# TIXhjq/ML_Function

Measured on AMD Instinct MI355X. Metric: samples/sec fwd+bwd xDeepFM-CIN B=4096,F=39,K=16, higher is better.
Workload: dtype f32

## Files before the change

### ml_function_amd/csrc/cin.hip

```cpp
#include "cin_kernels.h"
#include "cin_tail.h"
#include "cin_launch.h"
#include "cin_qtail.h"
#include "cin_qsplit.h"
#include "cin_qmerge.h"

#include <stdlib.h>

namespace fil {

struct CinShape {
  int B, F, K, L;
  int H[kCinMaxL];
  int Hp(int l) const { return l == 0 ? F : H[l - 1]; }
  int HS(int l) const { return 128 * cdiv(H[l], 128); }
  int xps(int l) const { return l == 0 ? F : HS(l - 1); }
  long M() const { return (long)B * K; }
  int JT() const { return cin_jt_of(F); }
  int HSmax() const {
    int h = 0;
    for (int l = 0; l < L; ++l) h = std::max(h, HS(l));
    return h;
  }
};
// ... 224 lines not shown
  return w;
}
static int dz_periods(const CinShape& s, int l) { return cdiv(s.Hp(l), cin_dz_h_per_period(s.JT())); }
static size_t wz_floats(const CinShape& s) {
  const int jts = cin_jt_sym(s.F);
  size_t w = ((size_t)cdiv(s.F, cin_dz_h_per_period(jts)) * cin_dz_tiles_per_period(jts) + 1) * 32 * s.HS(0);
  w = std::max(w, (size_t)s.F * (s.F / 2 + 1) * s.H[0]);
  for (int l = 0; l < s.L; ++l) w = std::max(w, ((size_t)dz_periods(s, l) * cin_dz_tiles_per_period(s.JT()) + 1) * 32 * s.HS(l));
  return w;
}
static int pool_chunks(const CinShape& s, int l) { return std::max(chunks_of(s.H[l]), l > 0 ? chunks_of(s.H[l - 1]) : 1); }
static size_t fwd_ws_bytes(const CinShape& s) {
  size_t t = 0;
  for (int l = 0; l < s.L; ++l) t += align_up((size_t)pool_chunks(s, l) * s.M() * sizeof(float), 256);
  t += align_up((size_t)s.Hp(s.L - 1) * s.F * sizeof(float), 256);
  t += align_up(wf_floats(s) * sizeof(float), 256);
  t += align_up((size_t)kCinMaxH * sizeof(float), 256);
  t += align_up(cin_x2_floats(s.M(), cin_x2_len(s.F)) * sizeof(float), 256);
  t += align_up((size_t)chunks_of(s.H[0]) * s.F * 2 * cin_jt_sym(s.F) * 128 * sizeof(float), 256);
  t += align_up(qsplit_wb_bytes(s), 256);
  return t;
}
static size_t dw_part_floats(const CinShape& s) {
  size_t pmax = 0;
  for (int l = 0; l < s.L; ++l) pmax = std::max(pmax, (size_t)dw_plan(s.M(), s.Hp(l) * s.F, s.H[l]).splits * s.Hp(l) * s.F * s.H[l]);
  const int csym = s.F * (s.F / 2 + 1);
  pmax = std::max(pmax, (size_t)dw_plan(s.M(), csym, s.H[0]).splits * csym * s.H[0]);
  pmax = std::max(pmax, (size_t)dw_plan(s.M(), csym + s.F, s.H[0]).splits * (csym + s.F) * s.H[0]);
  if (s.L == 3) pmax = std::max(pmax, (size_t)cin_dwq_plan(s.M(), csym + s.F, cu_count()).pairs * (csym + s.F) * 256);
  if (s.L == 3) pmax = std::max(pmax, (size_t)cin_dwqb_plan(s.M(), csym + s.F, cu_count()).splits * (csym + s.F) * 256);
  pmax = std::max(pmax, (size_t)dw_plan(s.M(), s.Hp(s.L - 1), s.F).splits * s.Hp(s.L - 1) * s.F);
  pmax = std::max(pmax, (size_t)dw_plan(s.M(), s.F, s.Hp(s.L - 1)).splits * s.Hp(s.L - 1) * s.F);
  const TailGeom g = tail_geom(s);
  if (g.on) {
    pmax = std::max(pmax, (size_t)tail_dw_plan(s.M(), g.C1).splits * g.C1 * g.JP + (size_t)cdiv(g.Cp, kTailPc) * g.Hq * s.F);
  }
  return pmax;
}
static size_t bwd_ws_bytes(const CinShape& s) {
  const size_t LK = (size_t)s.L * s.K;
  const size_t M = (size_t)s.M();
  size_t t = 0;
  t += align_up((size_t)s.B * LK * sizeof(float), 256);
  t += 2 * align_up(M * s.HSmax() * sizeof(float), 256);
  t += align_up(dw_part_floats(s) * sizeof(float), 256);
  const size_t nblk = (size_t)cdiv(std::max(1, s.B), kHeadChunk);
  const size_t ncol = (M + kColRows - 1) / kColRows;
  t += align_up(std::max(ncol * s.HSmax(), nblk * (LK + 1)) * sizeof(float), 256);
  const size_t cl = (size_t)std::max(s.Hp(s.L - 1), s.L == 3 ? s.H[0] : 0) * s.F;
  t += 2 * align_up(cl * sizeof(float), 256);
  t += align_up(wz_floats(s) * sizeof(float), 256);
  t += 2 * align_up(M * s.F * sizeof(float), 256);
  t += align_up((size_t)s.F * s.F * kCinMaxH * sizeof(float), 256);
  t += align_up(((M + 255) / 256 + 1) * kQtConst * sizeof(float), 256);
  t += align_up(((M + 255) / 256) * (LK + 1) * sizeof(float), 256);
  t += 2 * align_up(qsplit_wzb_bytes(s), 256);
  return t;
}

template <typename KernelT>
static void allow_lds(KernelT kernel, size_t sh) {
  if (sh > 48 * 1024) (void)hipFuncSetAttribute(reinterpret_cast<const void*>(kernel), hipFuncAttributeMaxDynamicSharedMemorySize, (int)sh);
}

}

using namespace fil;

extern "C" size_t fil_cin_saved_bytes(int B, int F, int K, int L, const int* H) {
  CinShape s;
  if (check_shape("fil_cin_saved_bytes", B, F, K, L, H, s) != FIL_OK || B == 0) return 0;
  return saved_bytes(s);
}

extern "C" size_t fil_cin_fwd_workspace_bytes(int B, int F, int K, int L, const int* H) {
  CinShape s;
  if (check_shape("fil_cin_fwd_workspace_bytes", B, F, K, L, H, s) != FIL_OK || B == 0) return 0;
  return fwd_ws_bytes(s);
}

extern "C" size_t fil_cin_bwd_workspace_bytes(int B, int F, int K, int L, const int* H) {
  CinShape s;
  if (check_shape("fil_cin_bwd_workspace_bytes", B, F, K, L, H, s) != FIL_OK || B == 0) return 0;
  return bwd_ws_bytes(s);
}

extern "C" int fil_cin_grad_ready_points(int B, int F, int K, int L, const int* H, int mode, int* point) {
  CinShape s;
  if (int rc = check_shape("fil_cin_grad_ready_points", B, F, K, L, H, s)) return rc;
  if (point == nullptr || mode < 0 || mode > 1023) return fail(FIL_ERR_ARG, "fil_cin_grad_ready_points: point == NULL or mode %d out of range", mode);
  if ((mode & kCinRetiredBits) != 0) return fail(FIL_ERR_UNSUPPORTED, "fil_cin_grad_ready_points: mode %d holds a retired bit (2: the split-bf16 experiment)", mode);
  if (B == 0) {
    for (int i = 0; i <= L; ++i) point[i] = 0;
    return 1;
  }
  int pt = 0, l = L - 1;
  point[L] = pt++;
  if (qmerge_used(s, mode, CinTune(mode))) {
    point[0] = point[L] = 0;
    pt = 1;
    point[1] = point[2] = pt++;
    return pt;
  }
  if (tail_used(s, mode)) {
    point[L - 1] = point[L - 2] = pt++;
    l = L - 3;
  }
// ... 337 lines not shown
    mode |= bits;
  }
  const bool xt_in = (mode & FIL_CIN_X_TRANSPOSED) != 0;
  const CinTune tune(mode);
  const bool tail = tail_used(s, mode);
  const bool qtail = qtail_used(s, mode, tune);
  const bool qmerge = qmerge_used(s, mode, tune);
  const bool qsplit = qsplit_used(s, mode, tune);
  const int qnp = qsplit_planes(mode);
  const TailGeom tg = tail_geom(s);
  mode &= 1;
  FIL_CIN_CHECK_ARG(W && dW && dbias);
  hipStream_t st = (hipStream_t)stream;
  const size_t LK = (size_t)L * K;
  auto ready = [&](int slot) {
    if (grad_ready_events != nullptr && grad_ready_events[slot] != nullptr) (void)hipEventRecord((hipEvent_t)grad_ready_events[slot], st);
  };
  if (B == 0) {
    for (int l = 0; l < L; ++l) {
      (void)hipMemsetAsync(dW[l], 0, (size_t)s.Hp(l) * F * H[l] * sizeof(float), st);
      (void)hipMemsetAsync(dbias[l], 0, (size_t)H[l] * sizeof(float), st);
    }
    if (output_dim == 1) {
      (void)hipMemsetAsync(ddense_w, 0, LK * sizeof(float), st);
      (void)hipMemsetAsync(ddense_b, 0, sizeof(float), st);
    }
    for (int l = 0; l <= L; ++l) ready(l);
    return FIL_OK;
  }
  FIL_CIN_CHECK_ARG(g && dx && saved && (x || !xt_in));
  FIL_CIN_CHECK_ARG(output_dim != 1 || (dense_w && pooled && ddense_w && ddense_b));
  if (workspace == nullptr || workspace_bytes < bwd_ws_bytes(s))
    return fail(FIL_ERR_WORKSPACE, "fil_cin_bwd: workspace %zu < %zu bytes", workspace_bytes, bwd_ws_bytes(s));
  const long M = s.M();
  const int JT = s.JT();
  Carver ws(workspace);
  float* dP = ws.take<float>((size_t)B * LK);
  float* Gbuf[2];
  Gbuf[0] = ws.take<float>((size_t)M * s.HSmax());
  Gbuf[1] = ws.take<float>((size_t)M * s.HSmax());
  float* part = ws.take<float>(dw_part_floats(s));
  const int nblk = cdiv(B, kHeadChunk);
  const int ncol = (int)((M + kColRows - 1) / kColRows);
  float* small = ws.take<float>(std::max((size_t)ncol * s.HSmax(), (size_t)nblk * (LK + 1)));
  const size_t cl = (size_t)s.Hp(L - 1) * F;
  const size_t cl_buf = (size_t)std::max(s.Hp(L - 1), L == 3 ? H[0] : 0) * F;
  float* wsum = ws.take<float>(cl_buf);
  float* vlast = ws.take<float>(cl_buf);
  float* Wz = ws.take<float>(wz_floats(s));
  float* dxT = ws.take<float>((size_t)M * F);
  float* gx0T = ws.take<float>((size_t)M * F);
  float* qt_dT = ws.take<float>((size_t)F * F * kCinMaxH);
  const int qt_ndc = (int)((M + 255) / 256);
  float* qt_dcpart = ws.take<float>((size_t)(qt_ndc + 1) * kQtConst);
  float* qt_hpart = ws.take<float>((size_t)qt_ndc * (LK + 1));
  u32x4* Wzb1 = reinterpret_cast<u32x4*>(ws.take<unsigned char>(qsplit_wzb_bytes(s)));
  u32x4* Wzb2 = reinterpret_cast<u32x4*>(ws.take<unsigned char>(qsplit_wzb_bytes(s)));

  Carver sv(const_cast<float*>(saved));
  const float* xT_own = sv.take<float>((size_t)M * F);
  const float* xT = xt_in ? x : xT_own;
  const float* maps[kCinMaxL];
  const float *tailY = nullptr, *tailUz = nullptr, *tailWsum = nullptr;
  const float *qtR = nullptr, *qtT = nullptr, *qtWsumL = nullptr, *qtCvec = nullptr, *qtWsumP = nullptr, *qtWsnP = nullptr, *qtWzT = nullptr;
  if (qtail) {
    maps[0] = sv.take<float>((size_t)M * s.HS(0));
    const float* q = sv.take<float>(qtail_saved_floats(s));
    qtR = q;
    qtT = qtR + (size_t)M * s.HS(0);
    qtWsumL = qtT + (size_t)F * F * H[0];
    qtCvec = qtWsumL + (size_t)H[1] * F;
    qtWsumP = qtCvec + 128;
    qtWsnP = qtWsumP + (size_t)H[0] * F;
    qtWzT = qtWsnP + qtail_wsn_floats(s);
  } else if (tail) {
    for (int l = 0; l < tg.p; ++l) maps[l] = sv.take<float>((size_t)M * s.HS(l));
    tailY = sv.take<float>((size_t)M * tg.JP);
    tailUz = sv.take<float>(tg.uz_floats + tg.uf_floats);
    tailWsum = sv.take<float>((size_t)tg.Hq * F);
  } else {
    for (int l = 0; l + 1 < L; ++l) maps[l] = sv.take<float>((size_t)M * s.HS(l));
  }

  const float* dPsrc = g;
  if (output_dim == 1 && qmerge) {
    dPsrc = dP;
  } else if (output_dim == 1) {
    ProfScope ps("cin_head_bwd", st);
    hipLaunchKernelGGL(cin_head_bwd_kernel, dim3(nblk), dim3(256), 0, st, g, dense_w, pooled, dP, small, B, (int)LK, kHeadChunk);
    if (!tail) hipLaunchKernelGGL(cin_reduce_kernel, dim3(cdiv((int)LK + 1, 64)), dim3(256), 0, st, small, ddense_w, (long)(LK + 1), nblk, ddense_b, (long)LK);
    FIL_CHECK_LAUNCH();
    dPsrc = dP;
  }
  if (!tail) ready(L);

  int cur = 0;
  int ltop = L - 1;
  bool dx_started = false;
  bool have_gx0 = false;
  bool wz_prepacked = false;
  bool qm_joined = false;
  if (qmerge) {
    const int p = tg.p, lL = L - 1, Hpp = tg.Hpp, Hq = tg.Hq, HS0 = s.HS(0);
    FIL_CIN_CHECK_ARG(bias && W[0] && W[p] && W[lL] && bias[p] && dW[0] && dW[p] && dW[lL] && dbias[0] && dbias[p] && dbias[lL]);
    const float* xpT = maps[p - 1];
    const int xps = s.xps(p);
    const float* dPp = dPsrc + (size_t)p * K;
// ... 15 lines not shown
      allow_lds(cin_qtail_xe_kernel<3>, sh);
      allow_lds(cin_qtail_xe_kernel<1>, sh);
      const int np = (int)std::min<long>(((long)tiles0 * 32 * HS0 + 255) / 256, 1024);
      const int nq2 = qsplit ? 2 * std::min(cdiv(tiles0 * 512, 256), 256) : 0;
      if (qnp == 1)
        hipLaunchKernelGGL(cin_qtail_xe_kernel<1>, dim3(qt_ndc + np + nq2), dim3(kXeThreads), sh, st, xT, dPL, dPp, (int)LK, K, xe, qt_dcpart, (int)M, F,
                           qt_ndc, output_dim == 1 ? g : nullptr, dense_w, pooled, dP, qt_hpart, (int)LK, lL, p, W[0], Wz, H[0], JTs, HS0, tiles0, np, qtT,
                           Hpp, Wzb1, Wzb2);
      else
        hipLaunchKernelGGL(cin_qtail_xe_kernel<3>, dim3(qt_ndc + np + nq2), dim3(kXeThreads), sh, st, xT, dPL, dPp, (int)LK, K, xe, qt_dcpart, (int)M, F,
                           qt_ndc, output_dim == 1 ? g : nullptr, dense_w, pooled, dP, qt_hpart, (int)LK, lL, p, W[0], Wz, H[0], JTs, HS0, tiles0, np, qtT,
                           Hpp, Wzb1, Wzb2);
    }
    FIL_CHECK_LAUNCH();
    {
      ProfScope ps("cin_last_bwd", st, 6.0 * (double)M * Hpp * F);
      cin_launch_last_bwd2(st, JT, xT, xpT, xps, qtWsumP, qtWsnP, dPp, (int)LK, dPprev, Gbuf[cur], HS0, dxT, (int)M, F, K, Hpp, qtR, HS0, dPL, small);
    }
    FIL_CHECK_LAUNCH();
    int dw_parts = 0;
    {
      ProfScope ps("cin_bwd_dw_q", st, algo1 + algo_tail, gemm_flops(M, 1, Cl, H[0]) + gemm_flops(M, 1, Cl, Hpp));
      if (qsplit) {
        const DwqbPlan bp = cin_dwqb_plan(M, Cl + F, cu_count());
        cin_launch_dwq_b(st, qnp, bp, Gbuf[cur], xpT, HS0, xe, XE, part, (int)M, F, symD);
        dw_parts = bp.splits;
      } else {
        const bool f4 = knobs().dwfold4 != 0;
        const DwqPlan dp = f4 ? cin_dwq_plan4(M, Cl + F, cu_count()) : cin_dwq_plan(M, Cl + F, cu_count());
        if (f4)
          hipLaunchKernelGGL((cin_dwq_kernel<kDwqDepth, 4>), dim3((dp.wgs + 7) / 8 * 8), dim3(kDwqThreads), 0, st, Gbuf[cur], xpT, HS0, xe, XE, part, (int)M, F,
                             symD, dp.rows_per_split, dp.splits, dp.ncol_full, dp.rem, dp.wgs_full, dp.wgs);
        else
          hipLaunchKernelGGL((cin_dwq_kernel<kDwqDepth, 2>), dim3((dp.wgs + 7) / 8 * 8), dim3(kDwqThreads), 0, st, Gbuf[cur], xpT, HS0, xe, XE, part, (int)M, F,
                             symD, dp.rows_per_split, dp.splits, dp.ncol_full, dp.rem, dp.wgs_full, dp.wgs);
        dw_parts = dp.pairs;
      }
    }
    FIL_CHECK_LAUNCH();
    {
      ProfScope ps("cin_reduce_dw", st);
      const int nb1 = cdiv(H[0], 64);
      const int nh = output_dim == 1 ? cdiv((int)LK + 1, 64) : 0;
      hipLaunchKernelGGL(cin_reduce_expand_q_kernel, dim3((Cl + F + 3) / 4 + nb1 + nh), dim3(256), 0, st, part, dw_parts, F, symD, H[0], Hpp, dW[0], qt_dT,
                         vlast, small, ncol, dbias[0], nb1, qt_hpart, qt_ndc, (int)LK, ddense_w, ddense_b);
    }
    FIL_CHECK_LAUNCH();
    ready(L);
    ready(0);
    {
      ProfScope ps("cin_tail_params", st);
      const size_t sh = cin_qtail_params_lds(F, Hq);
      allow_lds(cin_qtail_params_kernel, sh);
      float* dcfin = qt_dcpart + (size_t)qt_ndc * kQtConst;
      hipLaunchKernelGGL(cin_qtail_params_kernel, dim3(2 * Hpp + 1), dim3(256), sh, st, W[p], qtWsumL, qt_dT, vlast, dW[p], part, Hpp, F, Hq, qt_dcpart, qt_ndc,
                         dcfin);
      hipLaunchKernelGGL(cin_qtail_fill_kernel, dim3(cdiv(Hq * F, kQtFillCols)), dim3(kQtFillThreads), 0, st, part, Hpp, dcfin, bias[p], qtWsumL, dW[lL], dbias[p], dbias[lL], F, Hq,
                         tg.HL);
    }
    FIL_CHECK_LAUNCH();
    ready(lL);
    ready(p);
    const int NHMAX = HS0 / 2;
    if (NHMAX == 64 && knobs().dz2 != 0) {
      ProfScope ps("cin_bwd_dz_q", st, algo1 + algo_tail, gemm_flops(M, 1, Cl, H[0]) + gemm_flops(M, 1, Cl, Hpp));
      bool split_done = false;
      if (qsplit) {
        split_done = cin_launch_dz2_b(st, qnp, JTs, Gbuf[cur], xpT, HS0, dPL, (int)LK, K, Wzb1, Wzb2, xT, dxT, 1, (int)M, F, H[0], Hpp, periods, dx, qtCvec);
      }
      if (!split_done &&
          !cin_launch_dz2(st, JTs, Gbuf[cur], xpT, HS0, dPL, (int)LK, K, Wz, qtWzT, xT, dxT, 1, (int)M, F, H[0], Hpp, periods, dx, qtCvec))
        return fail(FIL_ERR_UNSUPPORTED, "fil_cin_bwd: no two-pass data-gradient kernel for JT=%d (F=%d)", JTs, F);
      qm_joined = true;
    } else {
      const bool two_waves = NHMAX == 64 && cin_dzs_two_waves(JTs) && tune.mb_forced != 2 && knobs().dzs_mb != 2;
      const int MBs = two_waves ? 1 : tune.mb_rows(M);
      const int ks = MBs != 1 ? 1 : tune.ksplit(M);
      const dim3 zgrid(ks == 4 ? cdiv((int)M, 32) : cdiv((int)M, 128 * MBs));
      {
        ProfScope ps("cin_bwd_dz_tail", st, algo_tail, gemm_flops(M, 1, Cl, Hpp));
        cin_launch_dz3_sym(st, MBs, JTs, NHMAX, zgrid, xpT, HS0, qtWzT, xT, gxR, dxR, 0, (int)M, F, Hpp, periods, ks);
      }
      FIL_CHECK_LAUNCH();
      {
        ProfScope ps("cin_bwd_dz_l1", st, algo1, gemm_flops(M, 1, Cl, H[0]));
        cin_launch_dz3_sym(st, MBs, JTs, NHMAX, zgrid, Gbuf[cur], HS0, Wz, xT, gx0T, dxT, 1, (int)M, F, H[0], periods, ks);
      }
      have_gx0 = true;
    }
    FIL_CHECK_LAUNCH();
    dx_started = true;
    ltop = -1;
  } else if (qtail) {
    const int p = tg.p, lL = L - 1, Hpp = tg.Hpp, Hq = tg.Hq, HS0 = s.HS(0);
    FIL_CIN_CHECK_ARG(bias && W[p] && W[lL] && bias[p] && dW[p] && dW[lL] && dbias[p] && dbias[lL]);
    const float* xpT = maps[p - 1];
    const int xps = s.xps(p);
    const float* dPp = dPsrc + (size_t)p * K;
    const float* dPL = dPsrc + (size_t)lL * K;
    const float* dPprev = dPsrc + (size_t)(p - 1) * K;
    const double algo = gemm_flops(M, Hpp, F, Hq) + gemm_flops(M, Hq, F, tg.HL);
    float* xs = Gbuf[1];
    float* gxR = xs + (size_t)M * (F + 1);
    float* dxR = gxR + (size_t)M * F;
    {
      ProfScope ps("cin_tail_a", st, (double)M * (F + 64) * sizeof(float));
      const size_t sh = (size_t)256 * (F + 3) * sizeof(float);
      allow_lds(cin_qtail_scale_kernel, sh);
      const int nh = output_dim == 1 ? cdiv((int)LK + 1, 64) : 0;
      FIL_CIN_CHECK_ARG(W[0]);
      const int JTs0 = cin_jt_sym(F);
      const int tiles0 = cdiv(F, cin_dz_h_per_period(JTs0)) * cin_dz_tiles_per_period(JTs0) + 1;
      const int np = (int)std::min<long>(((long)tiles0 * 32 * HS0 + 255) / 256, 1024);
      hipLaunchKernelGGL(cin_qtail_scale_kernel, dim3(qt_ndc + nh + np), dim3(256), sh, st, xT, dPL, dPp, (int)LK, K, xs, qt_dcpart, (int)M, F, qt_ndc, small,
                         ddense_w, ddense_b, (int)LK, nblk, nh, W[0], Wz, H[0], JTs0, HS0, tiles0);
      wz_prepacked = true;
    }
    FIL_CHECK_LAUNCH();
    ready(L);
    {
      ProfScope ps("cin_last_bwd", st, 6.0 * (double)M * Hpp * F);
      cin_launch_last_bwd2(st, JT, xT, xpT, xps, qtWsumP, qtWsnP, dPp, (int)LK, dPprev, Gbuf[cur], HS0, dxT, (int)M, F, K, Hpp, qtR, HS0, dPL, small);
    }
    FIL_CHECK_LAUNCH();
    const int symD = F / 2 + 1, Cl = F * symD;
    const int JTs = cin_jt_sym(F);
    {
      ProfScope ps("cin_bwd_dw_tail", st, algo, gemm_flops(M, 1, Cl, Hpp));
      const int parts = launch_dw3(st, dw_plan(M, Cl + F, Hpp), xpT, HS0, xT, xs, F + 1, part, M, F, F, Hpp, symD, F);
      const long nW = (long)Cl * Hpp, pstride = (long)(Cl + F) * Hpp;
      hipLaunchKernelGGL(cin_reduce_expand_sym_kernel, dim3((int)((nW + 63) / 64) + cdiv(F * Hpp, 64)), dim3(256), 0, st, part, qt_dT, F, symD, Hpp, parts,
                         pstride, vlast, (long)F * Hpp);
    }
    FIL_CHECK_LAUNCH();
    {
      ProfScope ps("cin_tail_params", st);
      const size_t sh = cin_qtail_params_lds(F, Hq);
      allow_lds(cin_qtail_params_kernel, sh);
      float* dcfin = qt_dcpart + (size_t)qt_ndc * kQtConst;
      hipLaunchKernelGGL(cin_qtail_params_kernel, dim3(2 * Hpp + 1), dim3(256), sh, st, W[p], qtWsumL, qt_dT, vlast, dW[p], part, Hpp, F, Hq, qt_dcpart, qt_ndc,
                         dcfin);
      hipLaunchKernelGGL(cin_qtail_fill_kernel, dim3(cdiv(Hq * F, kQtFillCols)), dim3(kQtFillThreads), 0, st, part, Hpp, dcfin, bias[p], qtWsumL, dW[lL], dbias[p], dbias[lL], F, Hq,
                         tg.HL);
    }
    FIL_CHECK_LAUNCH();
    ready(lL);
    ready(p);
    {
      const int periods = cdiv(F, cin_dz_h_per_period(JTs));
      ProfScope ps("cin_bwd_dz_tail", st, algo, gemm_flops(M, 1, Cl, Hpp));
      const int NHMAX = HS0 / 2;
      const bool two_waves = NHMAX == 64 && cin_dzs_two_waves(JTs) && tune.mb_forced != 2 && knobs().dzs_mb != 2;
      const int MBs = two_waves ? 1 : tune.mb_rows(M);
      const int ks = MBs != 1 ? 1 : tune.ksplit(M);
      cin_launch_dz3_sym(st, MBs, JTs, NHMAX, dim3(ks == 4 ? cdiv((int)M, 32) : cdiv((int)M, 128 * MBs)), xpT, HS0, qtWzT, xT, gxR, dxR, 0, (int)M, F, Hpp,
                         periods, ks);
    }
    FIL_CHECK_LAUNCH();
    dx_started = true;
    ltop = p - 1;
  } else if (tail) {
    const int p = tg.p, lL = L - 1;
    FIL_CIN_CHECK_ARG(bias && W[p] && W[lL] && bias[p] && dW[p] && dW[lL] && dbias[p] && dbias[lL]);
    const float* xpT = maps[p - 1];
    const int xps = s.xps(p);
    const double algo = gemm_flops(M, tg.Hpp, F, tg.Hq) + gemm_flops(M, tg.Hq, F, tg.HL);
    float* Apk = Gbuf[1];
    wz_prepacked = p == 1 && tune.sym && F >= 2;
    {
      ProfScope ps("cin_tail_a", st, (double)M * (F + 64) * sizeof(float));
      const int na = (int)std::min<long>((M * 16 * tg.NCB + 255) / 256, 4096);
      const int nh = output_dim == 1 ? cdiv((int)LK + 1, 64) : 0;
      int np = 0, JTs = 0, tiles0 = 0;
      if (wz_prepacked) {
        FIL_CIN_CHECK_ARG(W[0]);
        JTs = cin_jt_sym(F);
        tiles0 = cdiv(F, cin_dz_h_per_period(JTs)) * cin_dz_tiles_per_period(JTs) + 1;
        np = (int)std::min<long>(((long)tiles0 * 32 * s.HS(0) + 255) / 256, 1024);
      }
      hipLaunchKernelGGL(cin_tail_pre_kernel, dim3(na + nh + np), dim3(256), 0, st, xT, dPsrc, (int)LK, K, p, lL, Apk, (int)M, F, tg.NCB, na, small,
                         ddense_w, ddense_b, (int)LK, nblk, nh, W[0], Wz, H[0], JTs, s.HS(0), tiles0);
    }
    FIL_CHECK_LAUNCH();
    ready(L);
    const TailDwPlan tp = tail_dw_plan(M, tg.C1);
    {
      ProfScope ps("cin_bwd_dw_tail", st, algo, 2.0 * (double)M * tg.C1 * (F + 2));
      TailDwArgs a{Apk, xT, xpT, xps, part, (int)M, F, tg.Hpp, tg.JP, tp.rows_per_split, tp.blocks_x, tp.blocks_x * tp.splits, knobs().tail_settle != 0};
      cin_launch_tail_dw(st, tg.NCB, a);
    }
    FIL_CHECK_LAUNCH();
    {
      ProfScope ps("cin_tail_params", st);
      const int nblk_p = cdiv(tg.Cp, kTailPc);
      const int ldb = (tg.Hq + 3) & ~3;
      const size_t sh = ((size_t)(F + 1) * ldb + (size_t)tg.JP * (kTailPc + 4) + (size_t)kTailPc * ldb) * sizeof(float);
// ... 159 lines not shown
```

### ml_function_amd/csrc/cin_qtail.h

```cpp
#pragma once
#include "cin_kernels.h"
#include "cin_split.h"

namespace fil {

__device__ __forceinline__ void qt_stage(const float* __restrict__ src, float* dst, int n) {
  for (int i0 = threadIdx.x; i0 < n; i0 += 8 * 256) {
    float v[8];
#pragma unroll
    for (int u = 0; u < 8; ++u) v[u] = i0 + u * 256 < n ? src[i0 + u * 256] : 0.f;
#pragma unroll
    for (int u = 0; u < 8; ++u)
      if (i0 + u * 256 < n) dst[i0 + u * 256] = v[u];
  }
}
__device__ __forceinline__ void qt_stage_rows(const float* __restrict__ src, float* dst, int rows, int cols, int ld) {
  const int n = rows * cols;
  for (int i0 = threadIdx.x; i0 < n; i0 += 8 * 256) {
    float v[8];
#pragma unroll
    for (int u = 0; u < 8; ++u) v[u] = i0 + u * 256 < n ? src[i0 + u * 256] : 0.f;
#pragma unroll
    for (int u = 0; u < 8; ++u) {
      const int i = i0 + u * 256;
// ... 313 lines not shown
    }
  }
}

static __global__ __launch_bounds__(256) void cin_qtail_scale_kernel(const float* __restrict__ xT, const float* __restrict__ dPL,
                                                                     const float* __restrict__ dPp, int ldp, int K, float* __restrict__ xs,
                                                                     float* __restrict__ dcpart, int M, int F, int nscale,
                                                                     const float* __restrict__ hpart, float* __restrict__ ddw, float* __restrict__ ddb,
                                                                     int LK, int nhp, int nhead, const float* __restrict__ W0, float* __restrict__ Wz,
                                                                     int H0, int JTs, int HS0, int tiles0) {
  extern __shared__ __attribute__((aligned(16))) float smem[];
  if ((int)blockIdx.x >= nscale + nhead) {
    cin_pack_wz_sym_body(W0, Wz, F, H0, JTs, HS0, tiles0, blockIdx.x - nscale - nhead, gridDim.x - nscale - nhead);
    return;
  }
  if ((int)blockIdx.x >= nscale) {
    cin_reduce_body(hpart, ddw, (long)LK + 1, nhp, ddb, (long)LK, blockIdx.x - nscale);
    return;
  }
  const int ld = F + 3;
  const long m = (long)blockIdx.x * 256 + threadIdx.x;
  float* row = smem + threadIdx.x * ld;
  if (m < M) {
    const long b = m / K;
    const float dl = dPL[b * ldp + (m - b * K)], dp = dPp[b * ldp + (m - b * K)];
    for (int f = 0; f < F; ++f) {
      const float v = xT[m * F + f] * dl;
      xs[m * (F + 1) + f] = v;
      row[f] = v;
    }
    xs[m * (F + 1) + F] = dp;
    row[F] = dl;
    row[F + 1] = dp;
  } else {
    for (int f = 0; f < F + 2; ++f) row[f] = 0.f;
  }
  __syncthreads();
  __shared__ float cs[4][64];
  {
    const int f = threadIdx.x & 63, q = threadIdx.x >> 6;
    float t0 = 0.f, t1 = 0.f;
    if (f < F + 2) {
      for (int rr = 64 * q; rr < 64 * q + 64; rr += 2) {
        t0 += smem[rr * ld + f];
        t1 += smem[(rr + 1) * ld + f];
      }
    }
    cs[q][f] = t0 + t1;
  }
  __syncthreads();
  if (threadIdx.x < F + 2) dcpart[(long)blockIdx.x * kQtConst + threadIdx.x] = (cs[0][threadIdx.x] + cs[1][threadIdx.x]) + (cs[2][threadIdx.x] + cs[3][threadIdx.x]);
}

static __global__ __launch_bounds__(256) void cin_qtail_params_kernel(const float* __restrict__ Wp, const float* __restrict__ wsumL,
                                                                      const float* __restrict__ dT, const float* __restrict__ vT,
                                                                      float* __restrict__ dWp, float* __restrict__ partL, int Hpp, int F, int Hq,
                                                                      const float* __restrict__ dcpart, int ndc, float* __restrict__ dcfin) {
  extern __shared__ __attribute__((aligned(16))) float smem[];
  if ((int)blockIdx.x == 2 * Hpp) {
    float* red = smem;
    const int lane = threadIdx.x & 63, wave = threadIdx.x >> 6;
    float a0 = 0.f, a1 = 0.f, a2 = 0.f, a3 = 0.f;
    if (lane < F + 2) {
      int p = wave;
      for (; p + 60 < ndc; p += 64) {
        float u[16];
#pragma unroll
        for (int e = 0; e < 16; ++e) u[e] = dcpart[(long)(p + 4 * e) * kQtConst + lane];
#pragma unroll
        for (int e = 0; e < 16; e += 4) {
          a0 += u[e];
          a1 += u[e + 1];
          a2 += u[e + 2];
          a3 += u[e + 3];
        }
      }
      for (; p < ndc; p += 4) a0 += dcpart[(long)p * kQtConst + lane];
    }
    red[wave * 64 + lane] = (a0 + a1) + (a2 + a3);
    __syncthreads();
    if (wave == 0) dcfin[lane] = (red[lane] + red[64 + lane]) + (red[128 + lane] + red[192 + lane]);
    return;
  }
  const int h = blockIdx.x >> 1, phase = blockIdx.x & 1;
  const int FT = (F + 31) & ~31, HT = (Hq + 31) & ~31, FK16 = (F + 15) & ~15, ldd = FT + 1;
  float* dt = smem;
  float* op = dt + FT * ldd;
  const int nop = phase == 0 ? HT * ldd : FK16 * HT;
  const float* osrc = phase == 0 ? wsumL : Wp + (long)h * F * Hq;
  const int ocols = phase == 0 ? F : Hq, old = phase == 0 ? ldd : HT, on = F * Hq;
  const float rF = 1.f / (float)F, rO = 1.f / (float)ocols;
  constexpr int ND = 8, NO = 24;
  float dv[ND], ov[NO];
#pragma unroll
  for (int u = 0; u < ND; ++u) dv[u] = (int)threadIdx.x + u * 256 < F * F ? dT[(long)(threadIdx.x + u * 256) * Hpp + h] : 0.f;
#pragma unroll
  for (int u = 0; u < NO; ++u) ov[u] = (int)threadIdx.x + u * 256 < on ? osrc[threadIdx.x + u * 256] : 0.f;
  for (int i = threadIdx.x; i < FT * ldd + nop; i += 256) smem[i] = 0.f;
  __syncthreads();
  auto put_dt = [&](int i, float v) {
    const int fp = (int)(((float)i + 0.5f) * rF);
    dt[fp * ldd + (i - fp * F)] = v;
  };
  auto put_op = [&](int i, float v) {
    const int rr = (int)(((float)i + 0.5f) * rO);
    op[rr * old + (i - rr * ocols)] = v;
  };
#pragma unroll
  for (int u = 0; u < ND; ++u)
    if ((int)threadIdx.x + u * 256 < F * F) put_dt(threadIdx.x + u * 256, dv[u]);
#pragma unroll
  for (int u = 0; u < NO; ++u)
    if ((int)threadIdx.x + u * 256 < on) put_op(threadIdx.x + u * 256, ov[u]);
  for (int i = threadIdx.x + ND * 256; i < F * F; i += 256) put_dt(i, dT[(long)i * Hpp + h]);
  for (int i = threadIdx.x + NO * 256; i < on; i += 256) put_op(i, osrc[i]);
  __syncthreads();
  const int lane = threadIdx.x & 63, wave = threadIdx.x >> 6, r = lane & 31, half = lane >> 5;
  const bool two = F > 32;
  if (phase == 0) {
    for (int nt = wave; nt < (HT >> 5); nt += 4) {
      float v0[16], v1[16];
#pragma unroll
      for (int reg = 0; reg < 16; ++reg) {
        const int fp = mfma32_row(reg, half);
        v0[reg] = vT[(long)min(fp, F - 1) * Hpp + h];
        v1[reg] = two ? vT[(long)min(fp + 32, F - 1) * Hpp + h] : 0.f;
      }
      f32x16 a0, a1;
#pragma unroll
      for (int i = 0; i < 16; ++i) a0[i] = a1[i] = 0.f;
      const float* ar = dt + r * ldd + half;
      const float* br = op + (nt * 32 + r) * ldd + half;
      for (int k0 = 0; k0 < FK16; k0 += 16) {
        float fa[8], fb[8], fc[8];
#pragma unroll
        for (int u = 0; u < 8; ++u) {
          fa[u] = ar[k0 + 2 * u];
          fb[u] = br[k0 + 2 * u];
          fc[u] = two ? ar[32 * ldd + k0 + 2 * u] : 0.f;
        }
#pragma unroll
        for (int u = 0; u < 8; ++u) {
          a0 = mfma32(fa[u], fb[u], a0);
          if (two) a1 = mfma32(fc[u], fb[u], a1);
        }
      }
      const int n = nt * 32 + r;
#pragma unroll
      for (int reg = 0; reg < 16; ++reg) {
        const int fp = mfma32_row(reg, half);
        if (n < Hq && fp < F) dWp[((long)h * F + fp) * Hq + n] = v0[reg] + a0[reg];
        if (two && n < Hq && fp + 32 < F) dWp[((long)h * F + fp + 32) * Hq + n] = v1[reg] + a1[reg];
      }
    }
  } else {
    float* pl = partL + (long)h * Hq * F;
    for (int mt = wave; mt < (HT >> 5); mt += 4) {
      f32x16 a0, a1;
#pragma unroll
      for (int i = 0; i < 16; ++i) a0[i] = a1[i] = 0.f;
      const float* ar = op + half * HT + mt * 32 + r;
      const float* br = dt + half * ldd + r;
      for (int k0 = 0; k0 < FK16; k0 += 16) {
        float fa[8], fb[8], fc[8];
#pragma unroll
        for (int u = 0; u < 8; ++u) {
          fa[u] = ar[(k0 + 2 * u) * HT];
          fb[u] = br[(k0 + 2 * u) * ldd];
          fc[u] = two ? br[(k0 + 2 * u) * ldd + 32] : 0.f;
        }
#pragma unroll
        for (int u = 0; u < 8; ++u) {
          a0 = mfma32(fa[u], fb[u], a0);
          if (two) a1 = mfma32(fa[u], fc[u], a1);
        }
      }
#pragma unroll
      for (int reg = 0; reg < 16; ++reg) {
        const int n = mt * 32 + mfma32_row(reg, half);
        if (n < Hq && r < F) pl[n * F + r] = a0[reg];
        if (two && n < Hq && r + 32 < F) pl[n * F + r + 32] = a1[reg];
      }
    }
  }
}

inline size_t cin_qtail_params_lds(int F, int Hq) {
  const size_t FT = ((size_t)F + 31) & ~(size_t)31, HT = ((size_t)Hq + 31) & ~(size_t)31, FK16 = ((size_t)F + 15) & ~(size_t)15, ldd = FT + 1;
  const size_t fl = FT * ldd + (HT * ldd > FK16 * HT ? HT * ldd : FK16 * HT);
  return (fl > 256 ? fl : 256) * sizeof(float);
}

constexpr int kQtFillCols = 32, kQtFillThreads = 512;
static __global__ __launch_bounds__(kQtFillThreads) void cin_qtail_fill_kernel(const float* __restrict__ partL, int Hpp, const float* __restrict__ dcfin,
                                                                               const float* __restrict__ bias_p, const float* __restrict__ wsumL,
                                                                               float* __restrict__ dWL, float* __restrict__ dbias_p,
                                                                               float* __restrict__ dbias_L, int F, int Hq, int HL) {
  __shared__ float dc[kQtConst];
  __shared__ float red[16][kQtFillCols];
  __shared__ float val[kQtFillCols];
  const int col = threadIdx.x & 31, grp = threadIdx.x >> 5;
  if (threadIdx.x < kQtConst) dc[threadIdx.x] = (int)threadIdx.x < F + 2 ? dcfin[threadIdx.x] : 0.f;
  const int C = Hq * F;
  const int c = blockIdx.x * kQtFillCols + col;
  float t = 0.f;
  if (c < C) {
    int h = grp;
    for (; h + 112 < Hpp; h += 128) {
      float u[8];
#pragma unroll
      for (int e = 0; e < 8; ++e) u[e] = partL[(long)(h + 16 * e) * C + c];
      t += ((u[0] + u[1]) + (u[2] + u[3])) + ((u[4] + u[5]) + (u[6] + u[7]));
    }
    for (; h < Hpp; h += 16) t += partL[(long)h * C + c];
  }
  red[grp][col] = t;
  __syncthreads();
  if (grp == 0 && c < C) {
    float a = 0.f;
#pragma unroll
    for (int g = 0; g < 16; ++g) a += red[g][col];
    const int n = c / F, f = c - n * F;
    val[col] = a + bias_p[n] * dc[f];
  }
  __syncthreads();
  for (int i = threadIdx.x; i < kQtFillCols * HL; i += kQtFillThreads) {
    const int rr = i / HL, cc = i - rr * HL;
    const int cr = blockIdx.x * kQtFillCols + rr;
    if (cr < C) dWL[(long)cr * HL + cc] = val[rr];
  }
  if (blockIdx.x == 0) {
    for (int n = threadIdx.x; n < Hq; n += kQtFillThreads) {
      float u = dc[F + 1];
      for (int f = 0; f < F; ++f) u = fmaf(wsumL[n * F + f], dc[f], u);
      dbias_p[n] = u;
    }
    for (int n = threadIdx.x; n < HL; n += kQtFillThreads) dbias_L[n] = dc[F];
  }
}

}
```

Baseline: 5.713 million.

## Fuse qtail params and fill kernels into one owner-tiled launch

```diff
diff --git a/ml_function_amd/csrc/cin.hip b/ml_function_amd/csrc/cin.hip
--- a/ml_function_amd/csrc/cin.hip
+++ b/ml_function_amd/csrc/cin.hip
@@ -300,7 +300,7 @@
   t += align_up(wz_floats(s) * sizeof(float), 256);
   t += 2 * align_up(M * s.F * sizeof(float), 256);
   t += align_up((size_t)s.F * s.F * kCinMaxH * sizeof(float), 256);
-  t += align_up(((M + 255) / 256 + 1) * kQtConst * sizeof(float), 256);
+  t += align_up(((M + 255) / 256) * kQtConst * sizeof(float), 256);
   t += align_up(((M + 255) / 256) * (LK + 1) * sizeof(float), 256);
   t += 2 * align_up(qsplit_wzb_bytes(s), 256);
   return t;
@@ -744,7 +744,7 @@
   float* gx0T = ws.take<float>((size_t)M * F);
   float* qt_dT = ws.take<float>((size_t)F * F * kCinMaxH);
   const int qt_ndc = (int)((M + 255) / 256);
-  float* qt_dcpart = ws.take<float>((size_t)(qt_ndc + 1) * kQtConst);
+  float* qt_dcpart = ws.take<float>((size_t)qt_ndc * kQtConst);
   float* qt_hpart = ws.take<float>((size_t)qt_ndc * (LK + 1));
   u32x4* Wzb1 = reinterpret_cast<u32x4*>(ws.take<unsigned char>(qsplit_wzb_bytes(s)));
   u32x4* Wzb2 = reinterpret_cast<u32x4*>(ws.take<unsigned char>(qsplit_wzb_bytes(s)));
@@ -866,11 +866,8 @@
       ProfScope ps("cin_tail_params", st);
       const size_t sh = cin_qtail_params_lds(F, Hq);
       allow_lds(cin_qtail_params_kernel, sh);
-      float* dcfin = qt_dcpart + (size_t)qt_ndc * kQtConst;
-      hipLaunchKernelGGL(cin_qtail_params_kernel, dim3(2 * Hpp + 1), dim3(256), sh, st, W[p], qtWsumL, qt_dT, vlast, dW[p], part, Hpp, F, Hq, qt_dcpart, qt_ndc,
-                         dcfin);
-      hipLaunchKernelGGL(cin_qtail_fill_kernel, dim3(cdiv(Hq * F, kQtFillCols)), dim3(kQtFillThreads), 0, st, part, Hpp, dcfin, bias[p], qtWsumL, dW[lL], dbias[p], dbias[lL], F, Hq,
-                         tg.HL);
+      hipLaunchKernelGGL(cin_qtail_params_kernel, dim3(cin_qtail_param_wgs(F, Hq, Hpp)), dim3(kQtParamThreads), sh, st, W[p], qtWsumL, qt_dT, vlast, dW[p], Hpp, F, Hq,
+                         qt_dcpart, qt_ndc, bias[p], dW[lL], dbias[p], dbias[lL], tg.HL);
     }
     FIL_CHECK_LAUNCH();
     ready(lL);
@@ -951,11 +948,8 @@
       ProfScope ps("cin_tail_params", st);
       const size_t sh = cin_qtail_params_lds(F, Hq);
       allow_lds(cin_qtail_params_kernel, sh);
-      float* dcfin = qt_dcpart + (size_t)qt_ndc * kQtConst;
-      hipLaunchKernelGGL(cin_qtail_params_kernel, dim3(2 * Hpp + 1), dim3(256), sh, st, W[p], qtWsumL, qt_dT, vlast, dW[p], part, Hpp, F, Hq, qt_dcpart, qt_ndc,
-                         dcfin);
-      hipLaunchKernelGGL(cin_qtail_fill_kernel, dim3(cdiv(Hq * F, kQtFillCols)), dim3(kQtFillThreads), 0, st, part, Hpp, dcfin, bias[p], qtWsumL, dW[lL], dbias[p], dbias[lL], F, Hq,
-                         tg.HL);
+      hipLaunchKernelGGL(cin_qtail_params_kernel, dim3(cin_qtail_param_wgs(F, Hq, Hpp)), dim3(kQtParamThreads), sh, st, W[p], qtWsumL, qt_dT, vlast, dW[p], Hpp, F, Hq,
+                         qt_dcpart, qt_ndc, bias[p], dW[lL], dbias[p], dbias[lL], tg.HL);
     }
     FIL_CHECK_LAUNCH();
     ready(lL);
diff --git a/ml_function_amd/csrc/cin_qtail.h b/ml_function_amd/csrc/cin_qtail.h
--- a/ml_function_amd/csrc/cin_qtail.h
+++ b/ml_function_amd/csrc/cin_qtail.h
@@ -389,191 +389,227 @@
   if (threadIdx.x < F + 2) dcpart[(long)blockIdx.x * kQtConst + threadIdx.x] = (cs[0][threadIdx.x] + cs[1][threadIdx.x]) + (cs[2][threadIdx.x] + cs[3][threadIdx.x]);
 }
 
-static __global__ __launch_bounds__(256) void cin_qtail_params_kernel(const float* __restrict__ Wp, const float* __restrict__ wsumL,
-                                                                      const float* __restrict__ dT, const float* __restrict__ vT,
-                                                                      float* __restrict__ dWp, float* __restrict__ partL, int Hpp, int F, int Hq,
-                                                                      const float* __restrict__ dcpart, int ndc, float* __restrict__ dcfin) {
+constexpr int kQtParamThreads = 1024;
+constexpr int kQtStageLd = 65;
+inline int cin_qtail_param_owners(int F, int Hq) { return ((Hq + 31) / 32) * ((F + 31) / 32); }
+inline int cin_qtail_param_wgs(int F, int Hq, int Hpp) { return cin_qtail_param_owners(F, Hq) + (Hpp + 3) / 4; }
+static __global__ __launch_bounds__(kQtParamThreads) void cin_qtail_params_kernel(const float* __restrict__ Wp, const float* __restrict__ wsumL,
+                                                                                  const float* __restrict__ dT, const float* __restrict__ vT,
+                                                                                  float* __restrict__ dWp, int Hpp, int F, int Hq,
+                                                                                  const float* __restrict__ dcpart, int ndc,
+                                                                                  const float* __restrict__ bias_p, float* __restrict__ dWL,
+                                                                                  float* __restrict__ dbias_p, float* __restrict__ dbias_L, int HL) {
   extern __shared__ __attribute__((aligned(16))) float smem[];
-  if ((int)blockIdx.x == 2 * Hpp) {
-    float* red = smem;
-    const int lane = threadIdx.x & 63, wave = threadIdx.x >> 6;
-    float a0 = 0.f, a1 = 0.f, a2 = 0.f, a3 = 0.f;
-    if (lane < F + 2) {
-      int p = wave;
-      for (; p + 60 < ndc; p += 64) {
-        float u[16];
-#pragma unroll
-        for (int e = 0; e < 16; ++e) u[e] = dcpart[(long)(p + 4 * e) * kQtConst + lane];
-#pragma unroll
-        for (int e = 0; e < 16; e += 4) {
-          a0 += u[e];
-          a1 += u[e + 1];
-          a2 += u[e + 2];
-          a3 += u[e + 3];
+  const int nfs = (F + 31) >> 5, nown = ((Hq + 31) >> 5) * nfs;
+  if ((int)blockIdx.x < nown) {
+    const int nt = blockIdx.x / nfs, fs = blockIdx.x - nt * nfs;
+    const int lane = threadIdx.x & 63, g = threadIdx.x >> 6, r = lane & 31, half = lane >> 5;
+    float* stage = smem;
+    float* red = stage + 2 * 64 * kQtStageLd;
+    float* dcr = red + 16 * 1024;
+    float* dc = dcr + 256;
+    if (g < 4) {
+      float a0 = 0.f, a1 = 0.f, a2 = 0.f, a3 = 0.f;
+      if (lane < F + 2) {
+        int p = g;
+        for (; p + 60 < ndc; p += 64) {
+          float u[16];
+#pragma unroll
+          for (int e = 0; e < 16; ++e) u[e] = dcpart[(long)(p + 4 * e) * kQtConst + lane];
+#pragma unroll
+          for (int e = 0; e < 16; e += 4) {
+            a0 += u[e];
+            a1 += u[e + 1];
+            a2 += u[e + 2];
+            a3 += u[e + 3];
+          }
         }
-      }
-      for (; p < ndc; p += 4) a0 += dcpart[(long)p * kQtConst + lane];
-    }
-    red[wave * 64 + lane] = (a0 + a1) + (a2 + a3);
+        for (; p < ndc; p += 4) a0 += dcpart[(long)p * kQtConst + lane];
+      }
+      dcr[g * 64 + lane] = (a0 + a1) + (a2 + a3);
+    }
+    const int KS = (F + 1) >> 1;
+    const int npass = Hpp > 64 ? 2 : 1, nit = npass * KS;
+    const bool tree = g + 112 < Hpp;
+    const int n = nt * 32 + r;
+    const int srow = threadIdx.x >> 4, skk = srow >> 5, sfl = srow & 31, sh4 = (threadIdx.x & 15) * 4;
+    const int sf = fs * 32 + sfl;
+    const bool vec = (Hpp & 3) == 0;
+    auto ld_stage = [&](int it, float (&v)[4]) {
+      const int pass = it / KS, fp = 2 * (it - pass * KS) + skk, h0 = pass * 64 + sh4;
+      const bool ok = it < nit && fp < F && sf < F;
+      const float* src = dT + (long)(ok ? fp * F + sf : 0) * Hpp + h0;
+      if (ok && vec && h0 + 3 < Hpp) {
+        const float4 q = *reinterpret_cast<const float4*>(src);
+        v[0] = q.x, v[1] = q.y, v[2] = q.z, v[3] = q.w;
+      } else {
+#pragma unroll
+        for (int j = 0; j < 4; ++j) v[j] = ok && h0 + j < Hpp ? src[j] : 0.f;
+      }
+    };
+    auto st_stage = [&](int it, const float (&v)[4]) {
+      float* dst = stage + (it & 1) * 64 * kQtStageLd + srow * kQtStageLd + sh4;
+#pragma unroll
+      for (int j = 0; j < 4; ++j) dst[j] = v[j];
+    };
+    auto ld_a = [&](int it, float (&a)[4]) {
+      const int pass = it / KS, fp = 2 * (it - pass * KS) + half;
+#pragma unroll
+      for (int e = 0; e < 4; ++e) {
+        const int h = pass * 64 + g + 16 * e;
+        a[e] = it < nit && fp < F && n < Hq && h < Hpp ? Wp[((long)h * F + fp) * Hq + n] : 0.f;
+      }
+    };
+    float sv[4], an[4], ac[4];
+    ld_stage(0, sv);
+    ld_a(0, ac);
+    st_stage(0, sv);
     __syncthreads();
-    if (wave == 0) dcfin[lane] = (red[lane] + red[64 + lane]) + (red[128 + lane] + red[192 + lane]);
+    if (threadIdx.x < 64) dc[threadIdx.x] = (dcr[threadIdx.x] + dcr[64 + threadIdx.x]) + (dcr[128 + threadIdx.x] + dcr[192 + threadIdx.x]);
+    f32x16 u[4], t;
+#pragma unroll
+    for (int i = 0; i < 16; ++i) t[i] = 0.f;
+    int it = 0;
+    for (int pass = 0; pass < npass; ++pass) {
+#pragma unroll
+      for (int e = 0; e < 4; ++e)
+#pragma unroll
+        for (int i = 0; i < 16; ++i) u[e][i] = 0.f;
+      for (int ks = 0; ks < KS; ++ks, ++it) {
+        ld_stage(it + 1, sv);
+        ld_a(it + 1, an);
+        const float* br = stage + (it & 1) * 64 * kQtStageLd + (half * 32 + r) * kQtStageLd + g;
+        float fb[4];
+#pragma unroll
+        for (int e = 0; e < 4; ++e) fb[e] = br[16 * e];
+#pragma unroll
+        for (int e = 0; e < 4; ++e) u[e] = mfma32(ac[e], fb[e], u[e]);
+        st_stage(it + 1, sv);
+#pragma unroll
+        for (int e = 0; e < 4; ++e) ac[e] = an[e];
+        __syncthreads();
+      }
+      if (tree) {
+        if (pass == 0) t = (u[0] + u[1]) + (u[2] + u[3]);
+        else {
+          const f32x16 q = t + ((u[0] + u[1]) + (u[2] + u[3]));
+#pragma unroll
+          for (int i = 0; i < 16; ++i) t[i] = 0.f + q[i];
+        }
+      } else {
+#pragma unroll
+        for (int e = 0; e < 4; ++e)
+          if (pass * 64 + g + 16 * e < Hpp) t += u[e];
+      }
+    }
+#pragma unroll
+    for (int reg = 0; reg < 16; ++reg) red[g * 1024 + mfma32_row(reg, half) * 32 + r] = t[reg];
+    __syncthreads();
+    {
+      const int i = threadIdx.x, nl = i >> 5, fl = i & 31;
+      const int nn = nt * 32 + nl, f = fs * 32 + fl;
+      float a = 0.f;
+#pragma unroll
+      for (int w = 0; w < 16; ++w) a += red[w * 1024 + i];
+      red[i] = nn < Hq && f < F ? a + bias_p[nn] * dc[f] : 0.f;
+    }
+    __syncthreads();
+    const int nf = min(32, F - fs * 32);
+    for (int nl = 0; nl < 32 && nt * 32 + nl < Hq; ++nl) {
+      float* dst = dWL + ((long)(nt * 32 + nl) * F + fs * 32) * HL;
+      const int cnt = nf * HL;
+      if ((HL & 3) == 0 && (reinterpret_cast<uintptr_t>(dWL) & 15) == 0) {
+        for (int i4 = threadIdx.x; i4 < (cnt >> 2); i4 += kQtParamThreads) {
+          const float v = red[nl * 32 + (4 * i4) / HL];
+          reinterpret_cast<float4*>(dst)[i4] = make_float4(v, v, v, v);
+        }
+      } else {
+        for (int i = threadIdx.x; i < cnt; i += kQtParamThreads) dst[i] = red[nl * 32 + i / HL];
+      }
+    }
+    if (fs == 0 && (int)threadIdx.x < 32 && n < Hq) {
+      float b = dc[F + 1];
+      for (int f = 0; f < F; ++f) b = fmaf(wsumL[n * F + f], dc[f], b);
+      dbias_p[n] = b;
+    }
+    if (blockIdx.x == 0)
+      for (int i = threadIdx.x; i < HL; i += kQtParamThreads) dbias_L[i] = dc[F];
     return;
   }
-  const int h = blockIdx.x >> 1, phase = blockIdx.x & 1;
+  const int tid = threadIdx.x & 255, quad = threadIdx.x >> 8;
+  const int h = ((int)blockIdx.x - nown) * 4 + quad;
+  const bool live = h < Hpp;
+  const int hc = live ? h : Hpp - 1;
   const int FT = (F + 31) & ~31, HT = (Hq + 31) & ~31, FK16 = (F + 15) & ~15, ldd = FT + 1;
-  float* dt = smem;
-  float* op = dt + FT * ldd;
-  const int nop = phase == 0 ? HT * ldd : FK16 * HT;
-  const float* osrc = phase == 0 ? wsumL : Wp + (long)h * F * Hq;
-  const int ocols = phase == 0 ? F : Hq, old = phase == 0 ? ldd : HT, on = F * Hq;
-  const float rF = 1.f / (float)F, rO = 1.f / (float)ocols;
-  constexpr int ND = 8, NO = 24;
+  float* wl = smem;
+  float* dt = wl + HT * ldd + quad * FT * ldd;
+  float* vq = wl + HT * ldd + 4 * FT * ldd + quad * 64;
+  const int on = F * Hq;
+  const float rF = 1.f / (float)F;
+  constexpr int ND = 8, NO = 8;
   float dv[ND], ov[NO];
 #pragma unroll
-  for (int u = 0; u < ND; ++u) dv[u] = (int)threadIdx.x + u * 256 < F * F ? dT[(long)(threadIdx.x + u * 256) * Hpp + h] : 0.f;
-#pragma unroll
-  for (int u = 0; u < NO; ++u) ov[u] = (int)threadIdx.x + u * 256 < on ? osrc[threadIdx.x + u * 256] : 0.f;
-  for (int i = threadIdx.x; i < FT * ldd + nop; i += 256) smem[i] = 0.f;
+  for (int u = 0; u < ND; ++u) dv[u] = tid + u * 256 < F * F ? dT[(long)(tid + u * 256) * Hpp + hc] : 0.f;
+#pragma unroll
+  for (int u = 0; u < NO; ++u) ov[u] = (int)threadIdx.x + u * kQtParamThreads < on ? wsumL[threadIdx.x + u * kQtParamThreads] : 0.f;
+  const float vv = tid < F ? vT[(long)tid * Hpp + hc] : 0.f;
+  for (int i = threadIdx.x; i < HT * ldd + 4 * FT * ldd; i += kQtParamThreads) smem[i] = 0.f;
   __syncthreads();
   auto put_dt = [&](int i, float v) {
     const int fp = (int)(((float)i + 0.5f) * rF);
     dt[fp * ldd + (i - fp * F)] = v;
   };
-  auto put_op = [&](int i, float v) {
-    const int rr = (int)(((float)i + 0.5f) * rO);
-    op[rr * old + (i - rr * ocols)] = v;
+  auto put_wl = [&](int i, float v) {
+    const int rr = (int)(((float)i + 0.5f) * rF);
+    wl[rr * ldd + (i - rr * F)] = v;
   };
 #pragma unroll
   for (int u = 0; u < ND; ++u)
-    if ((int)threadIdx.x + u * 256 < F * F) put_dt(threadIdx.x + u * 256, dv[u]);
+    if (tid + u * 256 < F * F) put_dt(tid + u * 256, dv[u]);
 #pragma unroll
   for (int u = 0; u < NO; ++u)
-    if ((int)threadIdx.x + u * 256 < on) put_op(threadIdx.x + u * 256, ov[u]);
-  for (int i = threadIdx.x + ND * 256; i < F * F; i += 256) put_dt(i, dT[(long)i * Hpp + h]);
-  for (int i = threadIdx.x + NO * 256; i < on; i += 256) put_op(i, osrc[i]);
+    if ((int)threadIdx.x + u * kQtParamThreads < on) put_wl(threadIdx.x + u * kQtParamThreads, ov[u]);
+  if (tid < 64) vq[tid] = vv;
+  for (int i = tid + ND * 256; i < F * F; i += 256) put_dt(i, dT[(long)i * Hpp + hc]);
+  for (int i = threadIdx.x + NO * kQtParamThreads; i < on; i += kQtParamThreads) put_wl(i, wsumL[i]);
   __syncthreads();
-  const int lane = threadIdx.x & 63, wave = threadIdx.x >> 6, r = lane & 31, half = lane >> 5;
+  if (!live) return;
+  const int lane = tid & 63, wave = tid >> 6, r = lane & 31, half = lane >> 5;
   const bool two = F > 32;
-  if (phase == 0) {
-    for (int nt = wave; nt < (HT >> 5); nt += 4) {
-      float v0[16], v1[16];
-#pragma unroll
-      for (int reg = 0; reg < 16; ++reg) {
-        const int fp = mfma32_row(reg, half);
-        v0[reg] = vT[(long)min(fp, F - 1) * Hpp + h];
-        v1[reg] = two ? vT[(long)min(fp + 32, F - 1) * Hpp + h] : 0.f;
-      }
-      f32x16 a0, a1;
-#pragma unroll
-      for (int i = 0; i < 16; ++i) a0[i] = a1[i] = 0.f;
-      const float* ar = dt + r * ldd + half;
-      const float* br = op + (nt * 32 + r) * ldd + half;
-      for (int k0 = 0; k0 < FK16; k0 += 16) {
-        float fa[8], fb[8], fc[8];
-#pragma unroll
-        for (int u = 0; u < 8; ++u) {
-          fa[u] = ar[k0 + 2 * u];
-          fb[u] = br[k0 + 2 * u];
-          fc[u] = two ? ar[32 * ldd + k0 + 2 * u] : 0.f;
-        }
-#pragma unroll
-        for (int u = 0; u < 8; ++u) {
-          a0 = mfma32(fa[u], fb[u], a0);
-          if (two) a1 = mfma32(fc[u], fb[u], a1);
-        }
-      }
-      const int n = nt * 32 + r;
-#pragma unroll
-      for (int reg = 0; reg < 16; ++reg) {
-        const int fp = mfma32_row(reg, half);
-        if (n < Hq && fp < F) dWp[((long)h * F + fp) * Hq + n] = v0[reg] + a0[reg];
-        if (two && n < Hq && fp + 32 < F) dWp[((long)h * F + fp + 32) * Hq + n] = v1[reg] + a1[reg];
-      }
-    }
-  } else {
-    float* pl = partL + (long)h * Hq * F;
-    for (int mt = wave; mt < (HT >> 5); mt += 4) {
-      f32x16 a0, a1;
-#pragma unroll
-      for (int i = 0; i < 16; ++i) a0[i] = a1[i] = 0.f;
-      const float* ar = op + half * HT + mt * 32 + r;
-      const float* br = dt + half * ldd + r;
-      for (int k0 = 0; k0 < FK16; k0 += 16) {
-        float fa[8], fb[8], fc[8];
-#pragma unroll
-        for (int u = 0; u < 8; ++u) {
-          fa[u] = ar[(k0 + 2 * u) * HT];
-          fb[u] = br[(k0 + 2 * u) * ldd];
-          fc[u] = two ? br[(k0 + 2 * u) * ldd + 32] : 0.f;
-        }
-#pragma unroll
-        for (int u = 0; u < 8; ++u) {
-          a0 = mfma32(fa[u], fb[u], a0);
-          if (two) a1 = mfma32(fa[u], fc[u], a1);
-        }
-      }
-#pragma unroll
-      for (int reg = 0; reg < 16; ++reg) {
-        const int n = mt * 32 + mfma32_row(reg, half);
-        if (n < Hq && r < F) pl[n * F + r] = a0[reg];
-        if (two && n < Hq && r + 32 < F) pl[n * F + r + 32] = a1[reg];
-      }
+  for (int nt = wave; nt < (HT >> 5); nt += 4) {
+    f32x16 a0, a1;
+#pragma unroll
+    for (int i = 0; i < 16; ++i) a0[i] = a1[i] = 0.f;
+    const float* ar = dt + r * ldd + half;
+    const float* br = wl + (nt * 32 + r) * ldd + half;
+    for (int k0 = 0; k0 < FK16; k0 += 16) {
+      float fa[8], fb[8], fc[8];
+#pragma unroll
+      for (int u = 0; u < 8; ++u) {
+        fa[u] = ar[k0 + 2 * u];
+        fb[u] = br[k0 + 2 * u];
+        fc[u] = two ? ar[32 * ldd + k0 + 2 * u] : 0.f;
+      }
+#pragma unroll
+      for (int u = 0; u < 8; ++u) {
+        a0 = mfma32(fa[u], fb[u], a0);
+        if (two) a1 = mfma32(fc[u], fb[u], a1);
+      }
+    }
+    const int n = nt * 32 + r;
+#pragma unroll
+    for (int reg = 0; reg < 16; ++reg) {
+      const int fp = mfma32_row(reg, half);
+      if (n < Hq && fp < F) dWp[((long)h * F + fp) * Hq + n] = vq[fp] + a0[reg];
+      if (two && n < Hq && fp + 32 < F) dWp[((long)h * F + fp + 32) * Hq + n] = vq[fp + 32] + a1[reg];
     }
   }
 }
 
 inline size_t cin_qtail_params_lds(int F, int Hq) {
-  const size_t FT = ((size_t)F + 31) & ~(size_t)31, HT = ((size_t)Hq + 31) & ~(size_t)31, FK16 = ((size_t)F + 15) & ~(size_t)15, ldd = FT + 1;
-  const size_t fl = FT * ldd + (HT * ldd > FK16 * HT ? HT * ldd : FK16 * HT);
-  return (fl > 256 ? fl : 256) * sizeof(float);
-}
-
-constexpr int kQtFillCols = 32, kQtFillThreads = 512;
-static __global__ __launch_bounds__(kQtFillThreads) void cin_qtail_fill_kernel(const float* __restrict__ partL, int Hpp, const float* __restrict__ dcfin,
-                                                                               const float* __restrict__ bias_p, const float* __restrict__ wsumL,
-                                                                               float* __restrict__ dWL, float* __restrict__ dbias_p,
-                                                                               float* __restrict__ dbias_L, int F, int Hq, int HL) {
-  __shared__ float dc[kQtConst];
-  __shared__ float red[16][kQtFillCols];
-  __shared__ float val[kQtFillCols];
-  const int col = threadIdx.x & 31, grp = threadIdx.x >> 5;
-  if (threadIdx.x < kQtConst) dc[threadIdx.x] = (int)threadIdx.x < F + 2 ? dcfin[threadIdx.x] : 0.f;
-  const int C = Hq * F;
-  const int c = blockIdx.x * kQtFillCols + col;
-  float t = 0.f;
-  if (c < C) {
-    int h = grp;
-    for (; h + 112 < Hpp; h += 128) {
-      float u[8];
-#pragma unroll
-      for (int e = 0; e < 8; ++e) u[e] = partL[(long)(h + 16 * e) * C + c];
-      t += ((u[0] + u[1]) + (u[2] + u[3])) + ((u[4] + u[5]) + (u[6] + u[7]));
-    }
-    for (; h < Hpp; h += 16) t += partL[(long)h * C + c];
-  }
-  red[grp][col] = t;
-  __syncthreads();
-  if (grp == 0 && c < C) {
-    float a = 0.f;
-#pragma unroll
-    for (int g = 0; g < 16; ++g) a += red[g][col];
-    const int n = c / F, f = c - n * F;
-    val[col] = a + bias_p[n] * dc[f];
-  }
-  __syncthreads();
-  for (int i = threadIdx.x; i < kQtFillCols * HL; i += kQtFillThreads) {
-    const int rr = i / HL, cc = i - rr * HL;
-    const int cr = blockIdx.x * kQtFillCols + rr;
-    if (cr < C) dWL[(long)cr * HL + cc] = val[rr];
-  }
-  if (blockIdx.x == 0) {
-    for (int n = threadIdx.x; n < Hq; n += kQtFillThreads) {
-      float u = dc[F + 1];
-      for (int f = 0; f < F; ++f) u = fmaf(wsumL[n * F + f], dc[f], u);
-      dbias_p[n] = u;
-    }
-    for (int n = threadIdx.x; n < HL; n += kQtFillThreads) dbias_L[n] = dc[F];
-  }
-}
-
-}
+  const size_t FT = ((size_t)F + 31) & ~(size_t)31, HT = ((size_t)Hq + 31) & ~(size_t)31, ldd = FT + 1;
+  const size_t own = 2 * 64 * kQtStageLd + 16 * 1024 + 256 + 64;
+  return std::max(own, HT * ldd + 4 * FT * ldd + 4 * 64) * sizeof(float);
+}
+
+}
```

After: 5.264 million. 7.9% lower.
